# tczhangzhi/pytorch-distributed

Measured on AMD Instinct MI355X. Metric: ImageNet images/sec (ResNet-50 train step, whole job), higher is better.
Workload: dtype bf16; 1 GPU; model=resnet50, global_batch=3072, image_size=224, parallelism=dp1, style=ddp, hip_ext=True, hipgraph=False

## Files before the change

### amdtrain/ops/csrc/wgrad.hip

```cpp
#include "common.h"

namespace {

using bf16 = __hip_bfloat16;
using bf16x8 = __attribute__((ext_vector_type(8))) short;
using f32x4 = __attribute__((ext_vector_type(4))) float;
using u32x2 = __attribute__((ext_vector_type(2))) unsigned int;

constexpr int TN2_TPB = 256;
constexpr int GROUP_BYTES = 512;

__device__ __forceinline__ int xcd_swz_tn2(int bid, int nwg) {
  constexpr int NXCD = 8;
  if (nwg < NXCD) return bid;
  int xcd = bid % NXCD, idx = bid / NXCD;
  int q = nwg / NXCD, r = nwg % NXCD;
  return (xcd < r ? xcd * (q + 1) : r * (q + 1) + (xcd - r) * q) + idx;
}

struct TnGeom {
  int H, W, Hout, Wout, stride;
  int kh, kw, pad;
  int sw, pw;
};

struct TnRow {
  long n_off;
  int hb, wb;
};

__device__ __forceinline__ TnRow tn2_decode_row(long m, const TnGeom& g) {
  TnRow r;
  long t = m;
  const int wo = (int)(t % g.Wout); t /= g.Wout;
  const int ho = (int)(t % g.Hout); t /= g.Hout;
  r.n_off = t * (long)g.H * g.W;
  r.hb = ho * g.stride - g.pad;
  r.wb = wo * g.sw - g.pw;
  return r;
}

__device__ __forceinline__ long tn2_gather_tap(const TnRow& r, int tap,
                                               const TnGeom& g) {
  const int kh = g.kw == 3 ? tap / 3 : g.kw == 4 ? tap >> 2 : tap / g.kw;
  const int h = r.hb + kh;
  const int w = r.wb + tap - kh * g.kw;
  if (h < 0 || h >= g.H || w < 0 || w >= g.W) return -1;
  return r.n_off + (long)h * g.W + w;
}

__device__ __forceinline__ long tn2_gather_stride(long m, const TnGeom& g) {
  long t = m;
  const int wo = (int)(t % g.Wout); t /= g.Wout;
  const int ho = (int)(t % g.Hout); t /= g.Hout;
  return (t * g.H + (long)ho * g.stride) * g.W + (long)wo * g.stride;
}

template <int NCOLS>
__device__ __forceinline__ int st_byte(int m, int c) {
  const int sub = (m >> 5) * (NCOLS / 16) + (c >> 4);
  const int G = sub * 2 + ((m >> 2) & 1);
  return G * GROUP_BYTES + ((m >> 3) & 3) * 128 + (m & 3) * 32 + (c & 15) * 2;
}

template <int NCOLS, int MC>
constexpr int tile_bytes() {
  return (MC / 32) * (NCOLS / 16) * 2 * GROUP_BYTES;
}

template <int MODE, int NCOLS, int MC, int NWAVES = 4>
__device__ __forceinline__ void stage_tn2(
    const bf16* __restrict__ g, int ld, long m0, long M, int col0,
    int total_cols, int cin, const TnGeom& geo, const bf16* __restrict__ zp,
    bf16* lds) {
  const int t = threadIdx.x;
  const int wave = t / AMD_WAVE, lane = t % AMD_WAVE;
  constexpr int SUBTILES = (MC / 32) * (NCOLS / 16);
  const int r = lane >> 5, q = (lane >> 3) & 3, j = (lane >> 1) & 3;
  const int c_half = (lane & 1) * 8;
  const int mfrag = q * 8 + r * 4 + j;
  TnRow rows[MC / 32];
  if (MODE == 2) {
#pragma unroll
    for (int mb = 0; mb < MC / 32; ++mb) {
      const long m = m0 + mb * 32 + mfrag;
      rows[mb] = tn2_decode_row(m < M ? m : M - 1, geo);
    }
  }
#pragma unroll
  for (int ss = 0; ss < SUBTILES / NWAVES; ++ss) {
    const int s = ss * NWAVES + wave;
    static_assert((NCOLS / 16) % NWAVES == 0, "wave round spans m-blocks");
    const int mb = (ss * NWAVES) / (NCOLS / 16);
    const int cs = (s % (NCOLS / 16)) * 16;
    const int mloc = mb * 32 + mfrag;
    const long m = m0 + mloc;
    const int col = col0 + cs + c_half;
    const bf16* src = zp;
    if (m < M && col + 8 <= total_cols) {
      if (MODE == 0) {
        src = g + m * (long)ld + col;
      } else if (MODE == 1) {
        src = g + tn2_gather_stride(m, geo) * (long)ld + col;
      } else {
        const int tap = (cin & (cin - 1)) == 0 ? col >> (__ffs(cin) - 1)
                                               : col / cin;
        const long row = tn2_gather_tap(rows[mb], tap, geo);
        if (row >= 0) src = g + row * (long)ld + (col - tap * cin);
      }
    }
    __builtin_amdgcn_global_load_lds(
        (const __attribute__((address_space(1))) unsigned int*)src,
        (__attribute__((address_space(3))) unsigned int*)(
            (char*)lds + s * 1024 + lane * 16),
        16, 0, 0);
  }
}

template <int N>
__device__ __forceinline__ void vmcnt_wait() {
  if constexpr (N == 0) asm volatile("s_waitcnt vmcnt(0)" ::: "memory");
  else if constexpr (N == 2) asm volatile("s_waitcnt vmcnt(2)" ::: "memory");
  else if constexpr (N == 4) asm volatile("s_waitcnt vmcnt(4)" ::: "memory");
  else if constexpr (N == 5) asm volatile("s_waitcnt vmcnt(5)" ::: "memory");
  else if constexpr (N == 6) asm volatile("s_waitcnt vmcnt(6)" ::: "memory");
  else if constexpr (N == 8) asm volatile("s_waitcnt vmcnt(8)" ::: "memory");
  else if constexpr (N == 10)
    asm volatile("s_waitcnt vmcnt(10)" ::: "memory");
  else if constexpr (N == 12)
    asm volatile("s_waitcnt vmcnt(12)" ::: "memory");
  else if constexpr (N == 16)
    asm volatile("s_waitcnt vmcnt(16)" ::: "memory");
  else static_assert(N == 0, "unsupported vmcnt");
}

template <int OFF>
__device__ __forceinline__ bf16x8 tr_frag(unsigned addr) {
  u32x2 v0, v1;
  asm volatile(
      "ds_read_b64_tr_b16 %0, %2 offset:%3\n\t"
      "ds_read_b64_tr_b16 %1, %2 offset:%4"
      : "=&v"(v0), "=&v"(v1)
      : "v"(addr), "i"(OFF), "i"(OFF + GROUP_BYTES));
  union {
    unsigned int u[4];
    bf16x8 f;
  } pack;
  pack.u[0] = v0.x;
  pack.u[1] = v0.y;
  pack.u[2] = v1.x;
  pack.u[3] = v1.y;
  return pack.f;
}

template <int GMODE, int NW, int KW, int MC, int NBUF = 2, bool BAND = false>
__global__ void __launch_bounds__(NW * KW * 64, (NW * KW == 4 ? 2 : 1))
tn2_kernel(const bf16* __restrict__ dY, const bf16* __restrict__ X,
           float* __restrict__ parts, long M, int N, int K9, int Cin,
           TnGeom geo, int nbn, int nbk, int msplit,
           const bf16* __restrict__ zp) {
  constexpr int NWAVES = NW * KW;
  constexpr int NCY = NW * 64;
  constexpr int NCX = KW * 64;
  constexpr int KSTEPS = MC / 32;
  constexpr int LC = (MC / 32) * (NCY / 16 + NCX / 16) * 64 / (NW * KW * 64);
  __shared__ __align__(16) char Ys[NBUF][tile_bytes<NCY, MC>()];
  __shared__ __align__(16) char Xs[NBUF][tile_bytes<NCX, MC>()];

  const int tiles = nbn * nbk;
  const int bid = xcd_swz_tn2(blockIdx.x, tiles * msplit);
  const int tile = bid % tiles;
  const int mpart = bid / tiles;
  const int bn = tile / nbk, bk = tile % nbk;
  const int n0 = bn * NCY;
  const int k0 = BAND ? bk * Cin + n0 : bk * NCX;

  const long mchunks = (M + MC - 1) / MC;
  const long cpp = (mchunks + msplit - 1) / msplit;
  const long mc0 = (long)mpart * cpp;
  const long mc1 = min(mc0 + cpp, mchunks);

  const int t = threadIdx.x;
  const int wave = t / AMD_WAVE, lane = t % AMD_WAVE;
  const int wn = (wave / KW) * 64;
  const int wk = (wave % KW) * 64;
  const int fr = lane & 15, fq = lane >> 4;

  f32x4 acc[4][4];
#pragma unroll
  for (int i = 0; i < 4; ++i)
#pragma unroll
    for (int j = 0; j < 4; ++j) acc[i][j] = {0.f, 0.f, 0.f, 0.f};

  if (mc0 < mc1) {
    const unsigned ybase0 =
        (unsigned)(unsigned long long)(&Ys[0][0]) + lane * 8 +
        (wn / 16) * 2 * GROUP_BYTES;
    const unsigned xbase0 =
        (unsigned)(unsigned long long)(&Xs[0][0]) + lane * 8 +
        (wk / 16) * 2 * GROUP_BYTES;
    constexpr unsigned YB = tile_bytes<NCY, MC>();
    constexpr unsigned XB = tile_bytes<NCX, MC>();

    stage_tn2<0, NCY, MC, NWAVES>(dY, N, mc0 * MC, M, n0, N, Cin, geo, zp,
                                  (bf16*)Ys[0]);
    stage_tn2<GMODE, NCX, MC, NWAVES>(X, Cin, mc0 * MC, M, k0, K9, Cin, geo,
                                      zp, (bf16*)Xs[0]);
    if (NBUF >= 3 && mc0 + 1 < mc1) {
      stage_tn2<0, NCY, MC, NWAVES>(dY, N, (mc0 + 1) * MC, M, n0, N, Cin,
                                    geo, zp, (bf16*)Ys[1]);
      stage_tn2<GMODE, NCX, MC, NWAVES>(X, Cin, (mc0 + 1) * MC, M, k0, K9,
                                        Cin, geo, zp, (bf16*)Xs[1]);
      vmcnt_wait<LC>();
    } else {
      vmcnt_wait<0>();
    }
    __builtin_amdgcn_s_barrier();

    for (long mc = mc0; mc < mc1; ++mc) {
      const int cur = (int)((mc - mc0) % NBUF);
      const long pre = NBUF >= 3 ? mc + 2 : mc + 1;
      if (pre < mc1) {
        const int nxt = (int)((pre - mc0) % NBUF);
        stage_tn2<0, NCY, MC, NWAVES>(dY, N, pre * MC, M, n0, N, Cin, geo,
                                      zp, (bf16*)Ys[nxt]);
        stage_tn2<GMODE, NCX, MC, NWAVES>(X, Cin, pre * MC, M, k0, K9, Cin,
                                          geo, zp, (bf16*)Xs[nxt]);
      }
      const unsigned yb = ybase0 + cur * YB;
      const unsigned xb = xbase0 + cur * XB;
#pragma unroll
      for (int ks = 0; ks < KSTEPS; ++ks) {
        bf16x8 a[4], b[4];
#pragma unroll
        for (int i = 0; i < 4; ++i)
          a[i] = tr_frag<0>(yb + (ks * (NCY / 16) + i) * 2 * GROUP_BYTES);
#pragma unroll
        for (int j = 0; j < 4; ++j)
          b[j] = tr_frag<0>(xb + (ks * (NCX / 16) + j) * 2 * GROUP_BYTES);
        asm volatile("s_waitcnt lgkmcnt(0)" ::: "memory");
        __builtin_amdgcn_sched_barrier(0);
        __builtin_amdgcn_s_setprio(1);
#pragma unroll
        for (int i = 0; i < 4; ++i)
#pragma unroll
          for (int j = 0; j < 4; ++j)
            acc[i][j] = __builtin_amdgcn_mfma_f32_16x16x32_bf16(
                a[i], b[j], acc[i][j], 0, 0, 0);
        __builtin_amdgcn_s_setprio(0);
      }
      if (NBUF >= 3 && mc + 2 < mc1)
        vmcnt_wait<LC>();
      else
        vmcnt_wait<0>();
      __builtin_amdgcn_s_barrier();
    }
  }

  const int kout_cols = BAND ? 9 * NCX : K9;
  float* out = parts + (long)mpart * N * (long)kout_cols;
#pragma unroll
  for (int i = 0; i < 4; ++i)
#pragma unroll
    for (int j = 0; j < 4; ++j)
#pragma unroll
      for (int r = 0; r < 4; ++r) {
        const int n = n0 + wn + i * 16 + fq * 4 + r;
        const int klocal = wk + j * 16 + fr;
        const int k = BAND ? bk * NCX + klocal : k0 + klocal;
        if (n < N && (BAND || k < K9))
          out[(long)n * kout_cols + k] = acc[i][j][r];
      }
}

constexpr int TN2_FOLD = 16;

__global__ void __launch_bounds__(AMD_TPB)
tn2_collapse_kernel(const float* __restrict__ parts, float* __restrict__ out,
                    int nparts, int step, long NK) {
  const long nv = NK / 4;
  const int slot = blockIdx.x % step;
  for (long i = (long)(blockIdx.x / step) * blockDim.x + threadIdx.x; i < nv;
       i += (long)(gridDim.x / step) * blockDim.x) {
    f32x4 s = ((const f32x4*)(parts + (long)slot * NK))[i];
    for (int p = slot + step; p < nparts; p += step) {
      f32x4 v = ((const f32x4*)(parts + (long)p * NK))[i];
      s.x += v.x; s.y += v.y; s.z += v.z; s.w += v.w;
    }
    ((f32x4*)(out + (long)slot * NK))[i] = s;
  }
}

__global__ void tr16_probe_kernel(const short* __restrict__ in,
                                  short* __restrict__ out) {
  __shared__ short lds[256];
  for (int i = threadIdx.x; i < 256; i += blockDim.x) lds[i] = in[i];
  __syncthreads();
  if (threadIdx.x < 64) {
    const unsigned addr =
        (unsigned)(unsigned long long)(&lds[0]) + threadIdx.x * 8;
    u32x2 v;
    asm volatile("ds_read_b64_tr_b16 %0, %1 offset:0"
                 : "=&v"(v) : "v"(addr));
    asm volatile("s_waitcnt lgkmcnt(0)" ::: "memory");
    short4 s;
    __builtin_memcpy(&s, &v, 8);
    out[threadIdx.x * 4 + 0] = s.x;
    out[threadIdx.x * 4 + 1] = s.y;
    out[threadIdx.x * 4 + 2] = s.z;
    out[threadIdx.x * 4 + 3] = s.w;
  }
}

static at::Tensor tn2_zero_page(const at::Tensor& like) {
  static thread_local at::Tensor zp;
  if (!zp.defined() || zp.device() != like.device())
    zp = at::zeros({16}, like.options().dtype(at::kBFloat16));
  return zp;
}

template <int GMODE, int NW, int KW, int MC, int NBUF = 2>
void tn2_launch(const at::Tensor& dY, const at::Tensor& X, at::Tensor& out,
                long M, int N, int K9, int Cin, TnGeom geo, int target_blocks,
                hipStream_t stream) {
  const int nbn = (N + NW * 64 - 1) / (NW * 64);
  const int nbk = (K9 + KW * 64 - 1) / (KW * 64);
  const long tiles = (long)nbn * nbk;
  const long mchunks = (M + MC - 1) / MC;
  int msplit = (int)std::max<long>(
      1, std::min<long>(mchunks, target_blocks / tiles));
  auto zp = tn2_zero_page(dY);
  at::Tensor parts = out;
  if (msplit > 1)
    parts = at::empty({msplit, (long)N * K9}, out.options());
  tn2_kernel<GMODE, NW, KW, MC, NBUF>
      <<<(int)(tiles * msplit), NW * KW * 64, 0, stream>>>(
          (const bf16*)dY.const_data_ptr(), (const bf16*)X.const_data_ptr(),
          parts.data_ptr<float>(), M, N, K9, Cin, geo, nbn, nbk, msplit,
          (const bf16*)zp.const_data_ptr());
  CHECK_CUDA_OK();
  if (msplit > 1) {
    const long NK = (long)N * K9;
    TORCH_CHECK(NK % 4 == 0);
    const int nkgrid = amd_grid(NK / 4);
    if (msplit > 2 * TN2_FOLD) {
      auto folded = at::empty({TN2_FOLD, NK}, out.options());
      tn2_collapse_kernel<<<nkgrid * TN2_FOLD, AMD_TPB, 0, stream>>>(
          (const float*)parts.const_data_ptr(), folded.data_ptr<float>(),
          msplit, TN2_FOLD, NK);
      CHECK_CUDA_OK();
      tn2_collapse_kernel<<<nkgrid, AMD_TPB, 0, stream>>>(
          (const float*)folded.const_data_ptr(), out.data_ptr<float>(),
          TN2_FOLD, 1, NK);
      CHECK_CUDA_OK();
    } else {
      tn2_collapse_kernel<<<nkgrid, AMD_TPB, 0, stream>>>(
          (const float*)parts.const_data_ptr(), out.data_ptr<float>(), msplit,
          1, NK);
      CHECK_CUDA_OK();
    }
  }
}

}

at::Tensor tn2_wgrad(at::Tensor dY, at::Tensor X, long taps, long Nn, long H,
                     long W, long stride, long gmode, long kh, long kw,
                     long pad, long stride_w, long pad_w, long Hout,
                     long Wout) {
  TORCH_CHECK(dY.is_cuda() && dY.scalar_type() == at::kBFloat16 &&
              X.scalar_type() == at::kBFloat16);
  auto Yc = dY.contiguous();
  auto Xc = X.contiguous();
  const long M = Yc.size(0);
  const int N = (int)Yc.size(1);
  const int Cin = (int)Xc.size(1);
  const int K9 = (int)(taps * Cin);
  TORCH_CHECK(Cin % 8 == 0 && N % 8 == 0);
  TnGeom geo{0, 0, 0, 0, 1, 3, 3, 1, 1, 1};
  if (gmode == 1) {
    long Hout = (H + stride - 1) / stride, Wout = (W + stride - 1) / stride;
    TORCH_CHECK(M == Nn * Hout * Wout);
    geo = TnGeom{(int)H, (int)W, (int)Hout, (int)Wout, (int)stride, 1, 1, 0,
                 (int)stride, 0};
  } else if (gmode == 2) {
    const long sw = stride_w > 0 ? stride_w : stride;
    const long pw = pad_w >= 0 ? pad_w : pad;
    if (Hout <= 0) Hout = (H + 2 * pad - kh) / stride + 1;
    if (Wout <= 0) Wout = (W + 2 * pw - kw) / sw + 1;
    TORCH_CHECK(M == Nn * Hout * Wout && taps == kh * kw);
    TORCH_CHECK(Xc.size(0) == Nn * H * W);
    geo = TnGeom{(int)H, (int)W, (int)Hout, (int)Wout, (int)stride,
                 (int)kh, (int)kw, (int)pad, (int)sw, (int)pw};
  } else {
    TORCH_CHECK(M == Xc.size(0));
  }
  auto out = at::empty({(long)N, (long)K9}, Yc.options().dtype(at::kFloat));
  auto stream = at::cuda::getCurrentCUDAStream();
  const char* tb = std::getenv("AMDTRAIN_TN2_BLOCKS");
  const int target = tb ? atoi(tb) : 512;

  if (N < 128 && (K9 >= 256 || (gmode == 2 && Cin < 32))) {
    if (gmode == 2 && Cin >= 32 && std::getenv("AMDTRAIN_TN2_14") == nullptr)
      tn2_launch<2, 2, 2, 64>(Yc, Xc, out, M, N, K9, Cin, geo, target, stream);
    else if (gmode == 2 && std::getenv("AMDTRAIN_TN2_STEM22") != nullptr)
      tn2_launch<2, 2, 2, 64>(Yc, Xc, out, M, N, K9, Cin, geo, target, stream);
    else if (gmode == 2)
      tn2_launch<2, 1, 4, 32>(Yc, Xc, out, M, N, K9, Cin, geo, target, stream);
    else if (gmode == 1)
      tn2_launch<1, 2, 2, 64>(Yc, Xc, out, M, N, K9, Cin, geo, target, stream);
    else
      tn2_launch<0, 1, 4, 32>(Yc, Xc, out, M, N, K9, Cin, geo, target, stream);
  } else if (K9 < 128 && N >= 256 && gmode == 0) {
    tn2_launch<0, 4, 1, 32>(Yc, Xc, out, M, N, K9, Cin, geo, target, stream);
  } else {
    static const bool pipe3 = []() {
      const char* v = std::getenv("AMDTRAIN_TN2_PIPE3");
      return v && v[0] == '1';
    }();
    static const bool wide8 = []() {
      const char* v = std::getenv("AMDTRAIN_TN2_W8");
      return v && v[0] == '1';
    }();
    if ((wide8 || (gmode == 2 && K9 >= 4096)) && K9 % 256 == 0
        && gmode != 1) {
      if (gmode == 2)
        tn2_launch<2, 2, 4, 64>(Yc, Xc, out, M, N, K9, Cin, geo, target,
                                stream);
      else
        tn2_launch<0, 2, 4, 64>(Yc, Xc, out, M, N, K9, Cin, geo, target,
                                stream);
    } else if (pipe3) {
      if (gmode == 2)
        tn2_launch<2, 2, 2, 32, 3>(Yc, Xc, out, M, N, K9, Cin, geo, target,
                                   stream);
      else if (gmode == 1)
        tn2_launch<1, 2, 2, 32, 3>(Yc, Xc, out, M, N, K9, Cin, geo, target,
                                   stream);
      else
        tn2_launch<0, 2, 2, 32, 3>(Yc, Xc, out, M, N, K9, Cin, geo, target,
                                   stream);
    } else if (gmode == 2) {
      tn2_launch<2, 2, 2, 64>(Yc, Xc, out, M, N, K9, Cin, geo, target, stream);
    } else if (gmode == 1) {
      tn2_launch<1, 2, 2, 64>(Yc, Xc, out, M, N, K9, Cin, geo, target, stream);
    } else {
      tn2_launch<0, 2, 2, 64>(Yc, Xc, out, M, N, K9, Cin, geo, target, stream);
    }
  }
  return out;
}

at::Tensor tn2_wgrad_banded(at::Tensor dY, at::Tensor X, long Nn, long H,
                            long W, long stride) {
  TORCH_CHECK(dY.is_cuda() && dY.scalar_type() == at::kBFloat16 &&
              X.scalar_type() == at::kBFloat16);
  auto Yc = dY.contiguous();
  auto Xc = X.contiguous();
  const long M = Yc.size(0);
  const int N = (int)Yc.size(1);
  const int Cin = (int)Xc.size(1);
  TORCH_CHECK(N == Cin && N % 128 == 0);
  long Hout = (H + 2 - 3) / stride + 1, Wout = (W + 2 - 3) / stride + 1;
  TORCH_CHECK(M == Nn * Hout * Wout);
  TnGeom geo{(int)H, (int)W, (int)Hout, (int)Wout, (int)stride, 3, 3, 1,
             (int)stride, 1};
  auto out = at::empty({(long)N, (long)9 * 128},
                       Yc.options().dtype(at::kFloat));
  auto stream = at::cuda::getCurrentCUDAStream();
  const char* tb = std::getenv("AMDTRAIN_TN2_BLOCKS");
  const int target = tb ? atoi(tb) : 512;
  const int nbn = N / 128, nbk = 9;
  const long tiles = (long)nbn * nbk;
  const long mchunks = (M + 63) / 64;
  int msplit = (int)std::max<long>(
      1, std::min<long>(mchunks, target / tiles));
  auto zp = tn2_zero_page(Yc);
  at::Tensor parts = out;
  if (msplit > 1)
    parts = at::empty({msplit, (long)N * 9 * 128}, out.options());
  tn2_kernel<2, 2, 2, 64, 2, true>
      <<<(int)(tiles * msplit), TN2_TPB, 0, stream>>>(
          (const bf16*)Yc.const_data_ptr(), (const bf16*)Xc.const_data_ptr(),
          parts.data_ptr<float>(), M, N, 9 * Cin, Cin, geo, nbn, nbk, msplit,
          (const bf16*)zp.const_data_ptr());
  CHECK_CUDA_OK();
  if (msplit > 1) {
    const long NK = (long)N * 9 * 128;
    const int nkgrid = amd_grid(NK / 4);
    if (msplit > 2 * TN2_FOLD) {
      auto folded = at::empty({TN2_FOLD, NK}, out.options());
      tn2_collapse_kernel<<<nkgrid * TN2_FOLD, AMD_TPB, 0, stream>>>(
          (const float*)parts.const_data_ptr(), folded.data_ptr<float>(),
          msplit, TN2_FOLD, NK);
      CHECK_CUDA_OK();
      tn2_collapse_kernel<<<nkgrid, AMD_TPB, 0, stream>>>(
          (const float*)folded.const_data_ptr(), out.data_ptr<float>(),
          TN2_FOLD, 1, NK);
      CHECK_CUDA_OK();
    } else {
      tn2_collapse_kernel<<<nkgrid, AMD_TPB, 0, stream>>>(
          (const float*)parts.const_data_ptr(), out.data_ptr<float>(),
          msplit, 1, NK);
      CHECK_CUDA_OK();
    }
  }
  return out;
}

at::Tensor tr16_probe(at::Tensor in) {
  TORCH_CHECK(in.is_cuda() && in.scalar_type() == at::kShort &&
              in.numel() == 256);
  auto inc = in.contiguous();
  auto out = at::zeros({64, 4}, inc.options());
  auto stream = at::cuda::getCurrentCUDAStream();
  tr16_probe_kernel<<<1, 64, 0, stream>>>(
      (const short*)inc.const_data_ptr(), out.data_ptr<short>());
  CHECK_CUDA_OK();
  return out;
}
```

Baseline: 11050 images/sec.

## Walk gather addresses incrementally in weight-grad kernel and skip dead N columns

```diff
diff --git a/amdtrain/ops/csrc/wgrad.hip b/amdtrain/ops/csrc/wgrad.hip
--- a/amdtrain/ops/csrc/wgrad.hip
+++ b/amdtrain/ops/csrc/wgrad.hip
@@ -68,11 +68,11 @@
   return (MC / 32) * (NCOLS / 16) * 2 * GROUP_BYTES;
 }
 
-template <int MODE, int NCOLS, int MC, int NWAVES = 4>
+template <int MODE, int NCOLS, int MC, int NWAVES = 4, bool CUT = false>
 __device__ __forceinline__ void stage_tn2(
     const bf16* __restrict__ g, int ld, long m0, long M, int col0,
     int total_cols, int cin, const TnGeom& geo, const bf16* __restrict__ zp,
-    bf16* lds) {
+    bf16* lds, int ncut = 0) {
   const int t = threadIdx.x;
   const int wave = t / AMD_WAVE, lane = t % AMD_WAVE;
   constexpr int SUBTILES = (MC / 32) * (NCOLS / 16);
@@ -93,6 +93,7 @@
     static_assert((NCOLS / 16) % NWAVES == 0, "wave round spans m-blocks");
     const int mb = (ss * NWAVES) / (NCOLS / 16);
     const int cs = (s % (NCOLS / 16)) * 16;
+    if (CUT && col0 + cs >= ncut) continue;
     const int mloc = mb * 32 + mfrag;
     const long m = m0 + mloc;
     const int col = col0 + cs + c_half;
@@ -116,6 +117,121 @@
         16, 0, 0);
   }
 }
+
+
+struct TnStep {
+  int step;
+  int cw, ch;
+  int dhb, dwb;
+  int hhi, whi;
+  int hspan, wspan;
+  int nlive;
+};
+
+__device__ __forceinline__ unsigned tn2_range_mask(int b, int size, int k) {
+  const int lo = max(-b, 0);
+  const int hi = max(min(size - b, k), lo);
+  return (1u << hi) - (1u << lo);
+}
+
+template <int MODE, int NCOLS, int MC, int NWAVES>
+struct TnWalk {
+  static_assert(MODE == 1 || MODE == 2, "gather modes only");
+  static_assert((NCOLS / 16) % NWAVES == 0, "wave round spans m-blocks");
+  static constexpr int NRS = MC / 32;
+  static constexpr int NCS = (NCOLS / 16) / NWAVES;
+  static constexpr unsigned NEVER = 0x80000000u;
+
+  unsigned long long base[NRS];
+  int hb[NRS], wb[NRS];
+  long mrow;
+  unsigned toff[NCS], sel[NCS];
+
+  __device__ __forceinline__ void init(const bf16* g, int ld, long m0,
+                                       int col0, int total_cols, int cin,
+                                       const TnGeom& geo) {
+    const int lane = threadIdx.x % AMD_WAVE, wave = threadIdx.x / AMD_WAVE;
+    const int r = lane >> 5, q = (lane >> 3) & 3, j = (lane >> 1) & 3;
+    mrow = m0 + q * 8 + r * 4 + j;
+    const bool narrow = m0 + MC <= 0x7fffffffL;
+#pragma unroll
+    for (int mb = 0; mb < NRS; ++mb) {
+      long n;
+      int ho, wo;
+      if (narrow) {
+        const unsigned m = (unsigned)(mrow + mb * 32);
+        const unsigned t = m / (unsigned)geo.Wout;
+        wo = (int)(m - t * geo.Wout);
+        const unsigned nn = t / (unsigned)geo.Hout;
+        ho = (int)(t - nn * geo.Hout);
+        n = nn;
+      } else {
+        long t = mrow + mb * 32;
+        wo = (int)(t % geo.Wout); t /= geo.Wout;
+        ho = (int)(t % geo.Hout);
+        n = t / geo.Hout;
+      }
+      hb[mb] = ho * geo.stride - geo.pad;
+      wb[mb] = wo * geo.sw - geo.pw;
+      base[mb] = (unsigned long long)g +
+                 ((n * geo.H + hb[mb]) * geo.W + wb[mb]) * (long)ld * 2;
+    }
+#pragma unroll
+    for (int c = 0; c < NCS; ++c) {
+      const int col = col0 + (c * NWAVES + wave) * 16 + (lane & 1) * 8;
+      const bool in = col + 8 <= total_cols;
+      if (MODE == 1) {
+        toff[c] = col * 2;
+        sel[c] = in ? 1u : NEVER;
+      } else {
+        const int tap = col / cin;
+        const int kh = tap / geo.kw, kw = tap - kh * geo.kw;
+        toff[c] = ((kh * geo.W + kw) * ld + (col - tap * cin)) * 2;
+        sel[c] = in ? (1u << (kh & 15)) | (0x10000u << (kw & 15)) : NEVER;
+      }
+    }
+  }
+
+  __device__ __forceinline__ void stage(long M, const TnGeom& geo,
+                                        const TnStep& st,
+                                        const bf16* __restrict__ zp,
+                                        bf16* lds) {
+    const int lane = threadIdx.x % AMD_WAVE, wave = threadIdx.x / AMD_WAVE;
+    unsigned rmask[NRS];
+#pragma unroll
+    for (int mb = 0; mb < NRS; ++mb) {
+      const unsigned in =
+          MODE == 1 ? 1u
+                    : tn2_range_mask(hb[mb], geo.H, geo.kh) |
+                          tn2_range_mask(wb[mb], geo.W, geo.kw) << 16;
+      rmask[mb] = mrow + mb * 32 < M ? in : 0u;
+    }
+#pragma unroll
+    for (int ss = 0; ss < NRS * NCS; ++ss) {
+      const int mb = ss / NCS, c = ss % NCS;
+      const int s = ss * NWAVES + wave;
+      const unsigned long long a = base[mb] + toff[c];
+      const unsigned long long src =
+          (rmask[mb] & sel[c]) == sel[c] ? a : (unsigned long long)zp;
+      __builtin_amdgcn_global_load_lds(
+          (const __attribute__((address_space(1))) unsigned int*)src,
+          (__attribute__((address_space(3))) unsigned int*)(
+              (char*)lds + s * 1024 + lane * 16),
+          16, 0, 0);
+    }
+    mrow += MC;
+#pragma unroll
+    for (int mb = 0; mb < NRS; ++mb) {
+      wb[mb] += st.dwb;
+      const bool c1 = wb[mb] >= st.whi;
+      wb[mb] -= c1 ? st.wspan : 0;
+      hb[mb] += st.dhb + (c1 ? geo.stride : 0);
+      const bool c2 = hb[mb] >= st.hhi;
+      hb[mb] -= c2 ? st.hspan : 0;
+      base[mb] += (long)(st.step + (c1 ? st.cw : 0) + (c2 ? st.ch : 0));
+    }
+  }
+};
 
 template <int N>
 __device__ __forceinline__ void vmcnt_wait() {
@@ -153,16 +269,21 @@
   return pack.f;
 }
 
-template <int GMODE, int NW, int KW, int MC, int NBUF = 2, bool BAND = false>
-__global__ void __launch_bounds__(NW * KW * 64, (NW * KW == 4 ? 2 : 1))
+template <int GMODE, int NW, int KW, int MC, int NBUF = 2, bool BAND = false,
+          bool WALK = false>
+__global__ void __launch_bounds__(
+    NW * KW * 64,
+    (WALK && MC == 32 && NBUF == 2 ? 4 : NW * KW == 4 ? 2 : 1))
 tn2_kernel(const bf16* __restrict__ dY, const bf16* __restrict__ X,
            float* __restrict__ parts, long M, int N, int K9, int Cin,
            TnGeom geo, int nbn, int nbk, int msplit,
-           const bf16* __restrict__ zp) {
+           const bf16* __restrict__ zp, TnStep step) {
+  static_assert(!WALK || GMODE != 0, "plain rows have nothing to walk");
   constexpr int NWAVES = NW * KW;
   constexpr int NCY = NW * 64;
   constexpr int NCX = KW * 64;
   constexpr int KSTEPS = MC / 32;
+  constexpr bool NSKIP = WALK && NBUF == 2 && NW == 2 && KW == 2;
   constexpr int LC = (MC / 32) * (NCY / 16 + NCX / 16) * 64 / (NW * KW * 64);
   __shared__ __align__(16) char Ys[NBUF][tile_bytes<NCY, MC>()];
   __shared__ __align__(16) char Xs[NBUF][tile_bytes<NCX, MC>()];
@@ -202,15 +323,28 @@
     constexpr unsigned YB = tile_bytes<NCY, MC>();
     constexpr unsigned XB = tile_bytes<NCX, MC>();
 
-    stage_tn2<0, NCY, MC, NWAVES>(dY, N, mc0 * MC, M, n0, N, Cin, geo, zp,
-                                  (bf16*)Ys[0]);
-    stage_tn2<GMODE, NCX, MC, NWAVES>(X, Cin, mc0 * MC, M, k0, K9, Cin, geo,
-                                      zp, (bf16*)Xs[0]);
+    TnWalk<WALK ? GMODE : 1, NCX, MC, NWAVES> xw;
+    if constexpr (WALK) xw.init(X, Cin, mc0 * MC, k0, K9, Cin, geo);
+    auto stage_x = [&](long mch, char* dst) {
+      if constexpr (WALK)
+        xw.stage(M, geo, step, zp, (bf16*)dst);
+      else
+        stage_tn2<GMODE, NCX, MC, NWAVES>(X, Cin, mch * MC, M, k0, K9, Cin,
+                                          geo, zp, (bf16*)dst);
+    };
+
+    auto stage_y = [&](long mch, char* dst) {
+      stage_tn2<0, NCY, MC, NWAVES, NSKIP>(dY, N, mch * MC, M, n0, N, Cin, geo,
+                                           zp, (bf16*)dst, step.nlive);
+    };
+    const bool live =
+        !NSKIP || __builtin_amdgcn_readfirstlane(n0 + wn) < step.nlive;
+
+    stage_y(mc0, Ys[0]);
+    stage_x(mc0, Xs[0]);
     if (NBUF >= 3 && mc0 + 1 < mc1) {
-      stage_tn2<0, NCY, MC, NWAVES>(dY, N, (mc0 + 1) * MC, M, n0, N, Cin,
-                                    geo, zp, (bf16*)Ys[1]);
-      stage_tn2<GMODE, NCX, MC, NWAVES>(X, Cin, (mc0 + 1) * MC, M, k0, K9,
-                                        Cin, geo, zp, (bf16*)Xs[1]);
+      stage_y(mc0 + 1, Ys[1]);
+      stage_x(mc0 + 1, Xs[1]);
       vmcnt_wait<LC>();
     } else {
       vmcnt_wait<0>();
@@ -222,15 +356,14 @@
       const long pre = NBUF >= 3 ? mc + 2 : mc + 1;
       if (pre < mc1) {
         const int nxt = (int)((pre - mc0) % NBUF);
-        stage_tn2<0, NCY, MC, NWAVES>(dY, N, pre * MC, M, n0, N, Cin, geo,
-                                      zp, (bf16*)Ys[nxt]);
-        stage_tn2<GMODE, NCX, MC, NWAVES>(X, Cin, pre * MC, M, k0, K9, Cin,
-                                          geo, zp, (bf16*)Xs[nxt]);
+        stage_y(pre, Ys[nxt]);
+        stage_x(pre, Xs[nxt]);
       }
       const unsigned yb = ybase0 + cur * YB;
       const unsigned xb = xbase0 + cur * XB;
 #pragma unroll
       for (int ks = 0; ks < KSTEPS; ++ks) {
+        if (!live) break;
         bf16x8 a[4], b[4];
 #pragma unroll
         for (int i = 0; i < 4; ++i)
@@ -319,6 +452,39 @@
   return zp;
 }
 
+static bool tn2_walk_enabled() {
+  const char* v = std::getenv("AMDTRAIN_TN2_ADDR");
+  return !(v && v[0] == '0');
+}
+
+static bool tn2_nskip_enabled() {
+  const char* v = std::getenv("AMDTRAIN_TN2_NSKIP");
+  return !(v && v[0] == '0');
+}
+
+static bool tn2_make_step(const TnGeom& g, int MC, int ld, int N,
+                          TnStep* st) {
+  const long hw = (long)g.Hout * g.Wout;
+  const long dn = MC / hw, rem = MC % hw;
+  const long dh = rem / g.Wout, dw = rem % g.Wout;
+  const long step =
+      (dn * g.H * g.W + dh * g.stride * g.W + dw * g.sw) * ld * 2;
+  const long cw = ((long)g.stride * g.W - (long)g.Wout * g.sw) * ld * 2;
+  const long ch = ((long)g.H * g.W - (long)g.Hout * g.stride * g.W) * ld * 2;
+  const long tap = ((long)g.kh * g.W + g.kw + 1) * ld * 2;
+  const long lim = 1L << 29;
+  if (std::abs(step) >= lim || std::abs(cw) >= lim || std::abs(ch) >= lim ||
+      tap >= lim || g.kh > 15 || g.kw > 15 || g.pad > 15 || g.pw > 15 ||
+      g.pad < 0 || g.pw < 0)
+    return false;
+  *st = TnStep{(int)step, (int)cw, (int)ch,
+               (int)(dh * g.stride), (int)(dw * g.sw),
+               g.Hout * g.stride - g.pad, g.Wout * g.sw - g.pw,
+               g.Hout * g.stride, g.Wout * g.sw,
+               tn2_nskip_enabled() ? N : 0x7fffffff};
+  return true;
+}
+
 template <int GMODE, int NW, int KW, int MC, int NBUF = 2>
 void tn2_launch(const at::Tensor& dY, const at::Tensor& X, at::Tensor& out,
                 long M, int N, int K9, int Cin, TnGeom geo, int target_blocks,
@@ -333,11 +499,24 @@
   at::Tensor parts = out;
   if (msplit > 1)
     parts = at::empty({msplit, (long)N * K9}, out.options());
-  tn2_kernel<GMODE, NW, KW, MC, NBUF>
-      <<<(int)(tiles * msplit), NW * KW * 64, 0, stream>>>(
-          (const bf16*)dY.const_data_ptr(), (const bf16*)X.const_data_ptr(),
-          parts.data_ptr<float>(), M, N, K9, Cin, geo, nbn, nbk, msplit,
-          (const bf16*)zp.const_data_ptr());
+  TnStep st{};
+  bool walk = false;
+  if constexpr (GMODE != 0)
+    walk = tn2_walk_enabled() && tn2_make_step(geo, MC, Cin, N, &st);
+  auto launch = [&](auto kernel) {
+    kernel<<<(int)(tiles * msplit), NW * KW * 64, 0, stream>>>(
+        (const bf16*)dY.const_data_ptr(), (const bf16*)X.const_data_ptr(),
+        parts.data_ptr<float>(), M, N, K9, Cin, geo, nbn, nbk, msplit,
+        (const bf16*)zp.const_data_ptr(), st);
+  };
+  if constexpr (GMODE != 0) {
+    if (walk)
+      launch(tn2_kernel<GMODE, NW, KW, MC, NBUF, false, true>);
+    else
+      launch(tn2_kernel<GMODE, NW, KW, MC, NBUF>);
+  } else {
+    launch(tn2_kernel<GMODE, NW, KW, MC, NBUF>);
+  }
   CHECK_CUDA_OK();
   if (msplit > 1) {
     const long NK = (long)N * K9;
@@ -418,11 +597,12 @@
       const char* v = std::getenv("AMDTRAIN_TN2_PIPE3");
       return v && v[0] == '1';
     }();
-    static const bool wide8 = []() {
+    static const int w8 = []() {
       const char* v = std::getenv("AMDTRAIN_TN2_W8");
-      return v && v[0] == '1';
+      return v && v[0] == '1' ? 1 : v && v[0] == '0' ? 0 : -1;
     }();
-    if ((wide8 || (gmode == 2 && K9 >= 4096)) && K9 % 256 == 0
+    const bool wide8 = w8 == 1;
+    if ((wide8 || (w8 != 0 && gmode == 2 && K9 >= 4096)) && K9 % 256 == 0
         && gmode != 1) {
       if (gmode == 2)
         tn2_launch<2, 2, 4, 64>(Yc, Xc, out, M, N, K9, Cin, geo, target,
@@ -479,11 +659,18 @@
   at::Tensor parts = out;
   if (msplit > 1)
     parts = at::empty({msplit, (long)N * 9 * 128}, out.options());
-  tn2_kernel<2, 2, 2, 64, 2, true>
-      <<<(int)(tiles * msplit), TN2_TPB, 0, stream>>>(
-          (const bf16*)Yc.const_data_ptr(), (const bf16*)Xc.const_data_ptr(),
-          parts.data_ptr<float>(), M, N, 9 * Cin, Cin, geo, nbn, nbk, msplit,
-          (const bf16*)zp.const_data_ptr());
+  TnStep st{};
+  const bool walk = tn2_walk_enabled() && tn2_make_step(geo, 64, Cin, N, &st);
+  auto launch = [&](auto kernel) {
+    kernel<<<(int)(tiles * msplit), TN2_TPB, 0, stream>>>(
+        (const bf16*)Yc.const_data_ptr(), (const bf16*)Xc.const_data_ptr(),
+        parts.data_ptr<float>(), M, N, 9 * Cin, Cin, geo, nbn, nbk, msplit,
+        (const bf16*)zp.const_data_ptr(), st);
+  };
+  if (walk)
+    launch(tn2_kernel<2, 2, 2, 64, 2, true, true>);
+  else
+    launch(tn2_kernel<2, 2, 2, 64, 2, true>);
   CHECK_CUDA_OK();
   if (msplit > 1) {
     const long NK = (long)N * 9 * 128;
```

After: 11910 images/sec, median of 6. 7.9% higher.
